# RainBoltz/smore

Hardware: AMD Instinct MI355X
Metric: M edge-updates/sec (d=64, neg=5) (higher is better)
Workload: dtype f32; 1 GPU; LINE order-2 sampled negative-sampling SGD, config c4; vertices=10000000, edge_slots=400000000, dim=64, negative=5, scatter=hybrid, scatter_asked=hybrid, sync=none, parallelism=replicas1

## Files before the change

include/smore_hip.h:

```cpp
#ifndef SMORE_HIP_H
#define SMORE_HIP_H

#include <stddef.h>
#include <stdint.h>

#ifdef __cplusplus
extern "C" {
#endif

typedef struct smore_ctx smore_ctx;

#define SMORE_OK 0
#define SMORE_EINVAL 1
#define SMORE_EHIP 2
#define SMORE_ENOMEM 3
#define SMORE_ESTATE 4
#define SMORE_EIO 5

#define SMORE_VM_OUT_DEGREES 0
#define SMORE_VM_NO_DEGREES 1
#define SMORE_VM_DEGREES 2
#define SMORE_NM_DEGREES 0
#define SMORE_NM_IN_DEGREES 1
#define SMORE_NM_NO_DEGREES 2
// ... 58 lines not shown

int smore_train_edges_async(smore_ctx* ctx, int model, uint64_t begin, uint64_t count,
                            uint64_t total, int K, double alpha0, double reg, uint64_t seed,
                            int mode);
int smore_train_edges(smore_ctx* ctx, int model, uint64_t begin, uint64_t count,
                      uint64_t total, int K, double alpha0, double reg, uint64_t seed,
                      int mode);
int smore_set_hot_threshold(smore_ctx* ctx, double tau);
int smore_set_write_combine(smore_ctx* ctx, int rows, int flush_rounds);
int smore_write_combine_info(const smore_ctx* ctx, int* rows, int* flush_rounds);
int smore_hot_rows(const smore_ctx* ctx, int64_t* hot_w, int64_t* hot_c);
int smore_hot_row_ids(smore_ctx* ctx, int model, int K, int which, int64_t n, int32_t* ids);
int smore_skipped(smore_ctx* ctx, uint64_t* skipped);
float smore_last_kernel_ms(const smore_ctx* ctx);
int smore_last_mode(const smore_ctx* ctx);
int smore_copy_bandwidth(smore_ctx* ctx, uint64_t bytes, int reps, double* gbs);
int smore_last_phase_ms(const smore_ctx* ctx, float* draw_ms, float* update_ms, int* launches);

int smore_delta_begin(smore_ctx* ctx, const void* T, void* S, void* D, void* R, int64_t n);
int smore_delta_end(smore_ctx* ctx, void* T, void* S, const void* D, const void* R, float scale, int64_t n);
int smore_delta_cycle(smore_ctx* ctx, void* T, void* S, void* D, void* R, float scale, int64_t n);
int smore_delta_end_rows(smore_ctx* ctx, void* T, void* S, const void* D, const void* R, const void* scale,
                         int64_t rows, int64_t stride);
int smore_delta_cycle_rows(smore_ctx* ctx, void* T, void* S, void* D, void* R, const void* scale, int64_t rows,
                           int64_t stride);
int smore_source_parts(smore_ctx* ctx, int nparts, int64_t* bounds);
int smore_set_source_partition(smore_ctx* ctx, int nparts, int part);
int smore_row_rates(smore_ctx* ctx, int model, int K, int which, int64_t n, double* rate);
#define SMORE_SYNC_SUM 0
#define SMORE_SYNC_MEAN 1
// ... 194 lines not shown
```

smore_amd/_lib.py:

```python
import ctypes as C
import os

HERE = os.path.dirname(os.path.abspath(__file__))
LIB_PATH = os.environ.get("SMORE_LIB") or os.path.join(HERE, "lib", "libsmore_hip.so")

OK, EINVAL, EHIP, ENOMEM, ESTATE, EIO = range(6)
VM = {"out_degrees": 0, "no_degrees": 1, "degrees": 2}
NM = {"degrees": 0, "in_degrees": 1, "no_degrees": 2}
AT_VERTEX, AT_NEGATIVE, AT_CONTEXT = 0, 1, 2
W, CTX = 0, 1
MODEL = {"line2": 0, "line1": 1, "mf": 2, "bpr": 3, "census": 16}
SYNC = {"sum": 0, "mean": 1, "adaptive": 2}


def sync_rule(sync):
    if isinstance(sync, bool):
        return int(sync)
    return SYNC[sync]


MODE = {"hogwild": 0, "atomic": 1, "serial": 2, "hybrid": 3}
SCHED = {"replicas": 0, "blocks": 1}
SEM = {"cpp": 0, "go": 1}

# ... 35 lines not shown
        "smore_get_table": (i32, [P, i32, P, i64, i32]),
        "smore_table_device": (i32, [P, i32, C.POINTER(P), C.POINTER(i64)]),
        "smore_train_edges_async": (i32, [P, i32, u64, u64, u64, i32, dbl, dbl, u64, i32]),
        "smore_train_edges": (i32, [P, i32, u64, u64, u64, i32, dbl, dbl, u64, i32]),
        "smore_skipped": (i32, [P, C.POINTER(u64)]),
        "smore_set_hot_threshold": (i32, [P, dbl]),
        "smore_set_semantics": (i32, [P, i32]),
        "smore_set_write_combine": (i32, [P, i32, i32]),
        "smore_write_combine_info": (i32, [P, C.POINTER(i32), C.POINTER(i32)]),
        "smore_gen_powerlaw": (i32, [i64, i64, i32, dbl, u64, P, P]),
        "smore_hot_rows": (i32, [P, C.POINTER(i64), C.POINTER(i64)]),
        "smore_hot_row_ids": (i32, [P, i32, i32, i32, i64, P]),
        "smore_group_set_hot_exchange": (i32, [P, i64, i32]),
        "smore_last_kernel_ms": (C.c_float, [P]),
        "smore_last_mode": (i32, [P]),
        "smore_copy_bandwidth": (i32, [P, u64, i32, C.POINTER(C.c_double)]),
        "smore_last_phase_ms": (i32, [P, C.POINTER(C.c_float), C.POINTER(C.c_float), C.POINTER(i32)]),
        "smore_delta_begin": (i32, [P, P, P, P, P, i64]),
        "smore_delta_end": (i32, [P, P, P, P, P, C.c_float, i64]),
        "smore_delta_cycle": (i32, [P, P, P, P, P, C.c_float, i64]),
        "smore_delta_end_rows": (i32, [P, P, P, P, P, P, i64, i64]),
        "smore_delta_cycle_rows": (i32, [P, P, P, P, P, P, i64, i64]),
        "smore_row_rates": (i32, [P, i32, i32, i32, i64, P]),
        "smore_source_parts": (i32, [P, i32, P]),
        "smore_set_source_partition": (i32, [P, i32, i32]),
        "smore_exchange_set_adaptive": (i32, [P, i32, i32, dbl, dbl]),
        "smore_group_set_adaptive": (i32, [P, dbl]),
        "smore_group_set_partition": (i32, [P, i32]),
        "smore_group_set_walk_partition": (i32, [P, i32]),
        "smore_train_deepwalk": (i32, [P, u64, u64, i32, i32, i32, i32, dbl, u64, P, i32]),
# ... 118 lines not shown
```

smore_amd/csrc/capi.cpp:

```cpp
#include "hot_exchange.h"
#include "train_host.h"

#include <algorithm>
#include <chrono>
#include <cmath>
#include <cstdio>
#include <cstdlib>
#include <cstring>
#include <limits>
#include <string>
#include <vector>

using namespace smore_host;

extern "C" {

const char* smore_version(void) { return "smore_hip 0.1 (gfx950)"; }

int smore_create(int device, smore_ctx** out) {
    if (!out) return SMORE_EINVAL;
    *out = nullptr;
    smore_ctx* c = new smore_ctx();
    c->device = device;
    if (device < 0) {
// ... 19 lines not shown
}

void smore_destroy(smore_ctx* c) {
    if (!c) return;
    smore_exchange_release(c);
    if (c->device >= 0) {
        (void)hipSetDevice(c->device);
        (void)hipStreamSynchronize(c->stream);
    }
    dfree(c->d_offsets); dfree(c->d_targets); dfree(c->d_vtab); dfree(c->d_ntab); dfree(c->d_ctab);
    dfree(c->d_sig); dfree(c->d_skipped); dfree(c->d_work); dfree(c->d_warp_stats); dfree(c->d_field); dfree(c->d_hoprec_slots); dfree(c->d_hoprec_stats); dfree(c->d_skewopt_stats);
    dfree(c->d_table[0]); dfree(c->d_table[1]);

    dfree(c->d_order); dfree(c->d_walks); dfree(c->d_lens); dfree(c->d_tcum); dfree(c->d_wts); dfree(c->d_nbr_sorted); dfree(c->d_ntype); dfree(c->d_ttargets); dfree(c->d_toff); dfree(c->d_paths); dfree(c->d_path_off); dfree(c->d_t_off); dfree(c->d_t_tgt); dfree(c->d_t_ts); dfree(c->d_t_min); dfree(c->d_t_max); dfree(c->d_sh_hash); dfree(c->d_sh_ids);
    dfree(c->d_rec); dfree(c->d_vt32); dfree(c->d_ct16); dfree(c->d_split);
    dfree(c->d_pcount); dfree(c->d_poff); dfree(c->d_pairs); dfree(c->d_census[0]); dfree(c->d_census[1]);
    dfree(c->d_io_ids[0]); dfree(c->d_io_rows[0]); dfree(c->d_io_ids[1]); dfree(c->d_io_rows[1]);
    blocks_release(c);
    if (c->d_scan_tmp) (void)hipFree(c->d_scan_tmp);
    for (hipEvent_t e : c->phase_ev) (void)hipEventDestroy(e);
    if (c->ev0) (void)hipEventDestroy(c->ev0);
    if (c->ev1) (void)hipEventDestroy(c->ev1);
    if (c->own_stream) (void)hipStreamDestroy(c->own_stream);
    if (c->draw_stream) (void)hipStreamDestroy(c->draw_stream);
    for (hipEvent_t e : c->sync_ev) (void)hipEventDestroy(e);
    delete c;
}

const char* smore_last_error(const smore_ctx* c) { return c ? c->err.c_str() : "null context"; }

// ... 333 lines not shown
            if (e == hipSuccess) e = hipEventSynchronize(c->ev1);
            float ms = 0.0f;
            if (e == hipSuccess) e = hipEventElapsedTime(&ms, c->ev0, c->ev1);
            if (e == hipSuccess && ms > 0) best = std::max(best, 2.0 * (double)n16 * 16 * reps / (ms * 1e-3) / 1e9);
        }
    (void)hipFree(src);
    (void)hipFree(dst);
    c->timed = false;
    if (e != hipSuccess) return fail(c, SMORE_EHIP, hipGetErrorString(e));
    *gbs = best;
    return SMORE_OK;
}

int smore_last_mode(const smore_ctx* c) { return c ? c->last_mode : -1; }

float smore_last_kernel_ms(const smore_ctx* c) {
    if (!c || !c->timed) return -1.0f;
    float ms = -1.0f;
    if (hipEventSynchronize(c->ev1) != hipSuccess) return -1.0f;
    if (hipEventElapsedTime(&ms, c->ev0, c->ev1) != hipSuccess) return -1.0f;
    return ms;
}

int smore_deepwalk_order(int64_t V, int walk_times, uint64_t skip, int64_t* order) {
    if (V <= 0 || walk_times < 0 || !order) return SMORE_EINVAL;
    deepwalk_order(V, walk_times, skip, order);
    return SMORE_OK;
}

int smore_load_pretrain(smore_ctx* c, int which, const char* path) {
// ... 224 lines not shown
```

smore_amd/csrc/ctx.h:

```cpp
#pragma once
#include <hip/hip_runtime.h>

#include <algorithm>
#include <array>
#include <cmath>
#include <cstdlib>
#include <cstring>
#include <memory>
#include <string>
#include <vector>

#include "../../include/smore_hip.h"
#include "host_graph.h"
#include "train_kernels.h"

using namespace smore;

struct smore_ctx {
    int device = 0;
    hipStream_t stream = nullptr;
    hipStream_t own_stream = nullptr;
    hipStream_t draw_stream = nullptr;
    std::vector<hipEvent_t> sync_ev;
    std::string err;
// ... 56 lines not shown
    int32_t* d_t_tgt = nullptr;
    double* d_t_ts = nullptr;
    double* d_t_min = nullptr;
    double* d_t_max = nullptr;
    double t_min_time = 0.0, t_max_time = 0.0;
    bool has_temporal = false;
    int2* d_sh_hash = nullptr;
    int32_t* d_sh_ids = nullptr;
    int sh_rows = 0;
    int sh_max = 128, sh_flush = 0;
    int sh_flush_eff = 32;
    int sh_flush_w_eff = 0;
    int sh_lvl_eff[8] = {0, 0, 0, 0, 0, 0, 0, 0};
    int32_t* d_rec = nullptr;
    unsigned long long* d_split = nullptr;
    uint32_t* d_pcount = nullptr;
    uint64_t* d_poff = nullptr;
    size_t pair_walks = 0;
    void* d_scan_tmp = nullptr;
    size_t scan_tmp_bytes = 0;
    uint4* d_vt32 = nullptr;
    uint4* d_ct16 = nullptr;
    bool packed_ok = false;
    size_t rec_cap = 0;
    std::vector<hipEvent_t> phase_ev;
    int phase_n = 0;
    void* comm = nullptr;
    bool own_comm = false;
    bool local_comm = false;
    int nranks = 1, rank = 0;
// ... 213 lines not shown
```

smore_amd/csrc/edge_inst.h:

```cpp
#pragma once
#include "edge_kernels.h"

namespace smore {

template <int KMAX, int MODE>
const void* edge_symbol(int dpad, int model) {
    const int G = lanes_of(dpad), M = regs_of(dpad);
#define X(g, m)                                                                          \
    if (G == g && M == m) {                                                              \
        if (model == SMORE_BPR) {                                                        \
            if constexpr (KMAX == 5) return (const void*)edge_train_kernel<g, m, 5, MODE, 2>; \
            else return nullptr;                                                         \
        }                                                                                \
        return model == SMORE_LINE2 ? (const void*)edge_train_kernel<g, m, KMAX, MODE, 0> \
                                    : (const void*)edge_train_kernel<g, m, KMAX, MODE, 1>; \
    }
    SMORE_FOR_EACH_GM(X)
#undef X
    return nullptr;
}

template <int KMAX, int MODE>
const void* pair_symbol(int dpad, int) {
    const int G = lanes_of(dpad), M = regs_of(dpad);
// ... 9 lines not shown
```

smore_amd/csrc/edge_kernels.h:

```cpp
#pragma once
#include "train_kernels.h"

namespace smore {

#ifndef SMORE_WAVES_STORE
#define SMORE_WAVES_STORE 0
#endif
#ifndef SMORE_WAVES_ATOMIC
#define SMORE_WAVES_ATOMIC 0
#endif
#ifndef SMORE_WAVES_HYBRID
#define SMORE_WAVES_HYBRID 3
#endif
#ifndef SMORE_WAVES_BPR
#define SMORE_WAVES_BPR 0
#endif
constexpr int waves_of(int mode, int shared = 0) {
    return shared == 2 ? SMORE_WAVES_BPR
                       : mode == MODE_STORE ? SMORE_WAVES_STORE : mode == MODE_ATOMIC ? SMORE_WAVES_ATOMIC : SMORE_WAVES_HYBRID;
}

template <int MODE>
__device__ __forceinline__ bool scatter_atomic(int32_t tagged) {
    if constexpr (MODE == MODE_ATOMIC) return true;
// ... 461 lines not shown
        if (!(key & SH_WKEY)) continue;
        const float x = atomicExch(&sh.pend[i], 0.0f);
        if (x != 0.0f) unsafeAtomicAdd(Tw + (int64_t)(key & ~SH_WKEY) * dpad + (i - s * dpad), x);
    }
}

__device__ __forceinline__ float neg_scale_of(const EdgeArgs& a, uint64_t count) {
    if (a.neg_lo && a.neg_hi) {
        const uint64_t tot = *a.neg_hi - *a.neg_lo;
        return count > 0 && tot > 0 && a.neg_scale > 0.0f
                   ? (float)((double)a.neg_scale * (double)tot / (double)count) : 1.0f;
    }
    return a.neg_scale > 0.0f ? a.neg_scale : 1.0f;
}

template <int G, int M, int KMAX, int MODE, int SHARED>
__global__ void __launch_bounds__(256) __attribute__((amdgpu_waves_per_eu(waves_of(MODE, SHARED))))
edge_train_kernel(EdgeArgs a) {
    __shared__ float s_sig[1001];
    extern __shared__ float s_dyn[];
    int32_t* sh_ids = nullptr;
    const ShState sh = block_setup<MODE>(a, s_sig, s_dyn, sh_ids);

    const int lane = threadIdx.x & (G - 1);
    uint64_t rb = a.rec_base ? *a.rec_base : 0;
    uint64_t count = (a.count_dev ? *a.count_dev : a.count) - rb;
    const float nsc = neg_scale_of(a, count);
    if (a.part_n > 1) {
        const uint64_t lo = count * a.part_q / a.part_n, hi = count * (a.part_q + 1) / a.part_n;
        rb += lo;
        count = hi - lo;
    }
    const int32_t* const recs = a.rec + rb * (uint64_t)rec_width(KMAX);
// ... 103 lines not shown
#pragma unroll
            for (int q = 0; q < RW / 4; ++q) r[q] = i32x4{-1, -1, -1, -1};
            if (t < lim) {
                const i32x4* p = reinterpret_cast<const i32x4*>(recs + t * RW);
#pragma unroll
                for (int q = 0; q < RW / 4; ++q) r[q] = __builtin_nontemporal_load(p + q);
            }
        };
        i32x4 rr[RW / 4];
        Ids xa, xb;
        float wva[M], rowsa[KMAX + 1][M], wvb[M], rowsb[KMAX + 1][M];
        __shared__ uint64_t s_next;
        uint64_t ch_rounds = count / ((uint64_t)gridDim.x * gpb * 16u);
        ch_rounds = ch_rounds < 8 ? 8 : ch_rounds > CH_ROUNDS ? CH_ROUNDS : ch_rounds;
        if (a.pair_slice && !a.alpha_rec) ch_rounds = a.pair_slice;
        const uint64_t span = ch_rounds * gpb;
        auto grab = [&]() -> uint64_t {
            __syncthreads();
            if (threadIdx.x == 0) s_next = atomicAdd(a.work, 1ull) * span;
            __syncthreads();
            return s_next;
        };
        for (uint64_t c0 = grab(); c0 < count; c0 = grab()) {
            const uint64_t lim = c0 + span < count ? c0 + span : count;
            if constexpr (SHARED == 2) {
                uint64_t t = c0 + gib;
                load_rec(t, lim, rr);
                for (uint64_t r = c0; r < lim; r += gpb) {
                    t = r + gib;
                    decode(t, lim, rr, xa);
// ... 1 lines not shown
                    if (xa.live) {
                        int32_t id[KMAX + 1];
                        bool hot[KMAX + 1];
                        xa.ids(id);
                        xa.hots(hot);
                        gather_rows<G, M, KMAX>(a, lane, ev, xa.v(), id, shared, wva, rowsa);
                        if constexpr (KMAX == 5)
                            bpr_update_rows<G, M, KMAX, MODE>(a, s_sig, lane, ev, xa.v(), id,
                                                              scatter_atomic<MODE>(xa.w[0]), hot, xa.alpha, wva, rowsa,
                                                              sh);
                    }
                    maybe_flush();
                }
                continue;
            }
            uint64_t t = c0 + gib;
            load_rec(t, lim, rr);
            decode(t, lim, rr, xa);
            {
                int32_t id[KMAX + 1];
                xa.ids(id);
                gather_rows<G, M, KMAX>(a, lane, ev, xa.v(), id, shared, wva, rowsa);
            }
            load_rec(t + gpb, lim, rr);
            for (uint64_t r = c0; r < lim; r += gpb) {
                t = r + gib;
                decode(t + gpb, lim, rr, xb);
                load_rec(t + 2 * gpb, lim, rr);
                {
                    int32_t id[KMAX + 1];
// ... 153 lines not shown
```

smore_amd/csrc/train.cpp:

```cpp
#include "train_host.h"

#include <algorithm>
#include <cstdlib>
#include <cstring>
#include <string>
#include <thread>
#include <vector>

using namespace smore_host;

namespace smore_host {

int edge_grid(smore_ctx* c, const UpdateKernel& k, int mode, uint64_t count, bool leave_slot) {
    if (mode == SMORE_SERIAL) return 1;
    int per_cu = 0;
    if (!k.fn || hipOccupancyMaxActiveBlocksPerMultiprocessor(&per_cu, k.fn, 256, k.lds) != hipSuccess || per_cu < 1)
        per_cu = 1;
    if (leave_slot && per_cu > 1) per_cu -= 1;
    if (const char* e = getenv("SMORE_BLOCKS_PER_CU")) {
        const int cap = atoi(e);
        if (cap > 0 && cap < per_cu) per_cu = cap;
    }
    int64_t grid = (int64_t)c->cus * per_cu;
    if (const char* e = getenv("SMORE_MAX_BLOCKS")) {
// ... 140 lines not shown
        } else {
            a.K = K;
        }
    }
    if (model == SMORE_BPR && !go && mode == SMORE_HYBRID) {
        const char* e = getenv("SMORE_BPR_SCATTER");
        EdgeArgs t = a;
        t.sh_rows = 0;
        const int64_t Mb = (int64_t)edge_grid(c, UpdateFamily::Cpp, t) * (256 / lanes_of(c->dpad));
        const bool small = c->hot_tau < 0 && 16.0 * (double)Mb >= (double)c->g->V;
        if (!small && !(e && !strcmp(e, "tagged"))) a.mode = mode = SMORE_HOGWILD;
    }
    const char* bpr_comb = getenv("SMORE_BPR_COMBINE");
    const bool combine = mode == SMORE_HYBRID && (go || model != SMORE_BPR || (bpr_comb && atoi(bpr_comb) != 0));
    const int hot_model = go && model == SMORE_BPR ? SMORE_LINE2 : model;
    int grid;
    if ((rc = plan_record_launch(c, a, combine, fam, hot_model, go ? HOT_TAU_WALK : HOT_TAU_EDGE,
                                 EDGE_FLUSH_MAX, &grid)))
        return rc;
    const int RW = rec_width(kmax_of(a.K));
    uint64_t chunk_max = (uint64_t)1 << 27;
    if (const char* e = getenv("SMORE_DRAW_CHUNK")) chunk_max = std::max<uint64_t>(1024, strtoull(e, nullptr, 10));
    if (a.mode == SMORE_SERIAL) chunk_max = ((uint64_t)1 << 30) / (uint64_t)RW;
    const uint64_t chunk = std::min<uint64_t>(count, chunk_max);
    const int nch = (int)((count + chunk - 1) / chunk);
    const int nbuf = nch > 1 ? 2 : 1;
    if ((rc = ensure_cap(c, c->d_rec, c->rec_cap, chunk * RW * nbuf))) return rc;
    if ((rc = grow_events(c, c->phase_ev, 2 * (size_t)nch + 1))) return rc;
    if ((rc = grow_events(c, c->sync_ev, 2 * (size_t)nch))) return rc;
    if ((rc = ensure_packed(c))) return rc;
    const DevGraph dg = dev_graph(c);
    const bool split = mode == SMORE_HYBRID && !go && dg.vt32 && split_on();
    if (split && !c->d_split) HIPCHK(c, hipMalloc((void**)&c->d_split, 4 * sizeof(unsigned long long)));
    const char* leave_env = getenv("SMORE_DRAW_LEAVE");
    const bool leave = !leave_env || atoi(leave_env) != 0;
    const int ugrid = nch > 1 ? edge_grid(c, fam, a, leave) : grid;
    hipStream_t ds = nch > 1 ? c->draw_stream : c->stream;
    auto recbuf = [&](int k) { return c->d_rec + (size_t)(k % nbuf) * chunk * RW; };
    auto draw = [&](int k) -> int {
        const uint64_t b = (uint64_t)k * chunk, n = std::min<uint64_t>(chunk, count - b);
        if (k >= 2) HIPCHK(c, hipStreamWaitEvent(ds, c->sync_ev[2 * (k - 2) + 1], 0));
        if (go) HIPCHK(c, launch_go_draw(dg, c->d_tcum, c->go_unit_w, seed, begin + b, n, a.K, recbuf(k), c->d_skipped, ds));
        else if (split) {
            unsigned long long* cnt = c->d_split + 2 * (k % nbuf);
            HIPCHK(c, hipMemsetAsync(cnt, 0, 2 * sizeof(unsigned long long), ds));
            HIPCHK(c, launch_draw_split(dg, seed, begin + b, n, a.K, alpha0, total,
                                        model == SMORE_MF || model == SMORE_BPR ? 0 : 1, recbuf(k), c->d_skipped, cnt,
                                        ds));
        } else HIPCHK(c, launch_draw(dg, seed, begin + b, n, a.K, recbuf(k), c->d_skipped, ds));
        HIPCHK(c, hipEventRecord(c->sync_ev[2 * k], ds));
        return SMORE_OK;
    };
    HIPCHK(c, hipEventRecord(c->ev0, c->stream));
    HIPCHK(c, hipEventRecord(c->phase_ev[0], c->stream));
    if (ds != c->stream) HIPCHK(c, hipStreamWaitEvent(ds, c->phase_ev[0], 0));
    if ((rc = draw(0))) return rc;
    for (int k = 0; k < nch; ++k) {
        if (k + 1 < nch && (rc = draw(k + 1))) return rc;
        HIPCHK(c, hipStreamWaitEvent(c->stream, c->sync_ev[2 * k], 0));
        HIPCHK(c, hipEventRecord(c->phase_ev[2 * k + 1], c->stream));
        const uint64_t b = (uint64_t)k * chunk, n = std::min<uint64_t>(chunk, count - b);
        EdgeArgs ak = a;
        ak.begin = begin + b;
        ak.count = n;
        ak.rec = recbuf(k);
        HIPCHK(c, hipMemsetAsync(c->d_work, 0, sizeof(unsigned long long), c->stream));
        if (split) {
            unsigned long long* cnt = c->d_split + 2 * (k % nbuf);
            ak.alpha_rec = 2;
            ak.count_dev = reinterpret_cast<const uint64_t*>(cnt);
            HIPCHK(c, launch_update(update_kernel(fam, ak), ak, ugrid, c->stream));
            EdgeArgs ac = ak;
            ac.mode = SMORE_HOGWILD;
            ac.sh_rows = 0;
            ac.count_dev = nullptr;
            ac.rec_base = reinterpret_cast<const uint64_t*>(cnt);
            HIPCHK(c, hipMemsetAsync(c->d_work, 0, sizeof(unsigned long long), c->stream));
            HIPCHK(c, launch_update(update_kernel(fam, ac), ac, edge_grid(c, fam, ac), c->stream));
        } else HIPCHK(c, launch_update(update_kernel(fam, ak), ak, ugrid, c->stream));
        HIPCHK(c, hipEventRecord(c->phase_ev[2 * k + 2], c->stream));
// ... 429 lines not shown
```

smore_amd/csrc/train_kernels.h:

```cpp
#pragma once
#include <hip/hip_runtime.h>

#include <algorithm>
#include <cstdlib>

#include "../../include/smore_hip.h"
#include "device_common.h"

namespace smore {

enum { MODE_STORE = SMORE_HOGWILD, MODE_ATOMIC = SMORE_ATOMIC, MODE_HYBRID = SMORE_HYBRID };

struct EdgeArgs {
    DevGraph g;
    const float* sig;
    float* W;
    float* C;
    unsigned long long* skipped;
    const double* tcum;
    const int2* sh_hash;
    const int32_t* sh_ids;
    int sh_rows, sh_flush;
    int sh_flush_w;
    int sh_lvl[8];
    const int32_t* rec;
    const uint64_t* count_dev;
    const uint64_t* rec_base;
    unsigned long long* work;
    int alpha_rec;
    uint32_t pair_slice;
    float neg_scale;
    const uint64_t* neg_lo;
    const uint64_t* neg_hi;
    int w_plain;
    uint32_t part_q, part_n;
    int rec_edge;
    int w_comb;
    uint64_t begin, count, total, seed;
    double alpha0;
    float reg;
    int dpad, K, model, mode;
};

struct WalkArgs {
    const int64_t* order;
    uint64_t order_base;
    int32_t* walks;
    int32_t* lens;
    uint64_t walk_begin, nwalks, total_walks;
    int steps, window;
    int rule;
    int window_min;
// ... 16 lines not shown
    int sample_times;
    double jump;
};

int lanes_of(int dpad);
inline int regs_of(int dpad) {
    const int G = lanes_of(dpad);
    return 4 * ((dpad / 4 + G - 1) / G);
}
constexpr int rec_width(int kmax) {
    int r = 4;
    while (r < 2 + kmax) r <<= 1;
    return r;
}
constexpr uint64_t CH_ROUNDS = 128;
inline int kmax_of(int K) { return K <= 5 ? 5 : K <= 10 ? 10 : 20; }
hipError_t launch_delta_begin(const float* T, float* S, float* D, float* R, uint64_t n, int cus, hipStream_t st);
hipError_t launch_delta_end(float* T, float* S, const float* D, const float* R, float scale, uint64_t n, int cus,
                            hipStream_t st);
hipError_t launch_delta_cycle(float* T, float* S, float* D, float* R, float scale, uint64_t n, int cus,
                              hipStream_t st);
hipError_t launch_pair_count(const WalkArgs& w, uint64_t seed, uint32_t* count, hipStream_t st);
inline uint64_t pair_bound(int steps, int window, int rule = 0, int window_min = 0) {
    const uint64_t L = (uint64_t)steps + 1;
    if (rule == 1) return L * 2 * (uint64_t)std::max(1, window - window_min + 1);
    const uint64_t r = std::min<uint64_t>(2 * (uint64_t)window, L - 1);
    return L * r;
}
hipError_t scan_pair_counts(const uint32_t* count, uint64_t* off, uint64_t n, void** temp, size_t* temp_bytes,
                            hipStream_t st);
hipError_t launch_pair_emit(const DevGraph& g, const WalkArgs& w, uint64_t seed, int K, double alpha0,
                            const uint64_t* off, int32_t* rec, hipStream_t st);
hipError_t launch_pack(const DevGraph& g, uint64_t E, uint4* vt32, uint4* ct16, hipStream_t st);
hipError_t launch_draw_split(const DevGraph& g, uint64_t seed, uint64_t begin, uint64_t count, int K, double alpha0,
                             uint64_t total, int base, int32_t* rec, unsigned long long* skipped,
                             unsigned long long* counts, hipStream_t st);
hipError_t launch_draw(const DevGraph& g, uint64_t seed, uint64_t begin, uint64_t count, int K, int32_t* rec,
                       unsigned long long* skipped, hipStream_t st);
constexpr int SH_HASH = 256;
constexpr int32_t SH_WKEY = 1 << 30;
inline int sh_rows_max(int dpad) {
    static const int lds = [] {
        const char* e = getenv("SMORE_SH_LDS");
        const int v = e ? atoi(e) : 8192;
        return v > 0 ? v : 8192;
    }();
    const int r = lds / (dpad > 0 ? dpad : 1);
    return r < SH_HASH - 1 ? r : SH_HASH - 1;
}

inline size_t sh_lds_bytes(int sh_rows, int dpad) {
    return sh_rows > 0 ? SH_HASH * 8 + (size_t)sh_rows * 4 + (size_t)sh_rows * dpad * 4 : 0;
}
// ... 83 lines not shown
    X(Edge, MODE_ATOMIC, 5) X(Edge, MODE_ATOMIC, 10) X(Edge, MODE_ATOMIC, 20)       \
    X(Edge, MODE_HYBRID, 5) X(Edge, MODE_HYBRID, 10) X(Edge, MODE_HYBRID, 20)       \
    X(Pair, MODE_STORE, 5) X(Pair, MODE_STORE, 10)                                  \
    X(Pair, MODE_ATOMIC, 5) X(Pair, MODE_ATOMIC, 10)                                \
    X(Pair, MODE_HYBRID, 5) X(Pair, MODE_HYBRID, 10)                                \
    X(GoRec, MODE_STORE, 5) X(GoRec, MODE_STORE, 10)                                \
    X(GoRec, MODE_ATOMIC, 5) X(GoRec, MODE_ATOMIC, 10)                              \
    X(GoRec, MODE_HYBRID, 5) X(GoRec, MODE_HYBRID, 10)                              \
    X(GoPair, MODE_STORE, 5) X(GoPair, MODE_STORE, 10)                              \
    X(GoPair, MODE_ATOMIC, 5) X(GoPair, MODE_ATOMIC, 10)                            \
    X(GoPair, MODE_HYBRID, 5) X(GoPair, MODE_HYBRID, 10)                            \
    X(Warp, WARP_STORE, WARP_KMAX) X(Warp, WARP_ATOMIC, WARP_KMAX)                  \
    X(HopRec, MODE_STORE, HOPREC_KMAX) X(HopRec, MODE_ATOMIC, HOPREC_KMAX)          \
    X(SkewOpt, MODE_STORE, SKEWOPT_KMAX) X(SkewOpt, MODE_ATOMIC, SKEWOPT_KMAX)

template <KernelFamily F, int MODE, int KMAX>
const void* update_symbol(int dpad, int model);
#define X(F, MODE, KMAX) \
    template <>          \
    const void* update_symbol<KernelFamily::F, MODE, KMAX>(int dpad, int model);
SMORE_FOR_EACH_UPDATE_KERNEL(X)
#undef X
#define SMORE_UPDATE_INST(F, MODE, KMAX, ladder)                                          \
    namespace smore {                                                                     \
    template <>                                                                           \
    const void* update_symbol<KernelFamily::F, MODE, KMAX>(int dpad, int model) {         \
        return ladder<KMAX, MODE>(dpad, model);                                           \
    }                                                                                     \
    }

// ... 53 lines not shown
```

smore_amd/csrc/train_kernels.hip:

```cpp

#include "train_kernels.h"

namespace smore {

__global__ void sample_kernel(DevGraph g, uint64_t seed, uint64_t begin, uint64_t count, int K,
                              int bpr, int32_t* out) {
    const uint64_t t = (uint64_t)blockIdx.x * blockDim.x + threadIdx.x;
    if (t >= count) return;
    const uint64_t s = begin + t;
    const int nslot = bpr ? 14 : 4 + 2 * K;
    const int width = bpr ? 7 : 2 + K;
    int32_t* o = out + t * width;
    uint32_t w[4];
    uint32_t blk = 0xFFFFFFFFu;
    auto word = [&](int j) -> uint32_t {
        if ((uint32_t)(j >> 2) != blk) {
            blk = (uint32_t)(j >> 2);
            const uint4 b = philox_block(seed, 0, s, blk);
            w[0] = b.x; w[1] = b.y; w[2] = b.z; w[3] = b.w;
        }
        return w[j & 3];
    };
    (void)nslot;
    const int32_t v = untag(source_sample(g, word(0), word(1)));
// ... 38 lines not shown
    return nullptr;
}

static bool pair_path(const EdgeArgs& a) {
    return a.alpha_rec == 1 && a.mode != SMORE_SERIAL && a.K <= 10 && !a.rec_edge;
}

UpdateKernel update_kernel(UpdateFamily f, const EdgeArgs& a) {
    KernelFamily kf = KernelFamily::Edge;
    int kmax = kmax_of(a.K);
    switch (f) {
        case UpdateFamily::Cpp: kf = pair_path(a) ? KernelFamily::Pair : KernelFamily::Edge; break;
        case UpdateFamily::GoRec: kf = KernelFamily::GoRec; kmax = std::min(kmax, 10); break;
        case UpdateFamily::GoPair: kf = KernelFamily::GoPair; kmax = std::min(kmax, 10); break;
    }
    return {find_symbol(kf, a.mode, kmax, a.dpad, a.model),
            a.mode == SMORE_HYBRID ? sh_lds_bytes(a.sh_rows, a.dpad) : 0};
}

UpdateKernel update_kernel(const WarpArgs& a) {
    const int mode = a.mode == SMORE_ATOMIC ? SMORE_ATOMIC : SMORE_HOGWILD;
    return {find_symbol(KernelFamily::Warp, mode, WARP_KMAX, a.dpad, 0), 0};
}

UpdateKernel update_kernel(const HopRecArgs& a) {
    const int mode = a.mode == SMORE_ATOMIC ? SMORE_ATOMIC : SMORE_HOGWILD;
    return {find_symbol(KernelFamily::HopRec, mode, HOPREC_KMAX, a.dpad, 0), 0};
}

UpdateKernel update_kernel(const SkewOptArgs& a) {
    const int mode = a.mode == SMORE_ATOMIC ? SMORE_ATOMIC : SMORE_HOGWILD;
// ... 22 lines not shown
```

smore_amd/pronet.py:

```python
import ctypes as C

import numpy as np

from . import _lib
from ._lib import check, lib, ptr


class ProNet:

    def __init__(self, device=0, _ctx=None):
        self.ctx = C.c_void_p()
        self._owned = _ctx is None
        if _ctx is not None:
            self.ctx = C.c_void_p(_ctx)
        else:
            rc = lib.smore_create(int(device), C.byref(self.ctx))
            if rc != _lib.OK:
                raise _lib.SmoreError("smore_create(device=%d) failed with status %d" % (device, rc))
        self.device = device
        self.vertex_method = "out_degrees"
        self.negative_method = "degrees"
        self.dim = 0

    def close(self):
# ... 493 lines not shown
    def synchronize(self):
        self._chk(lib.smore_synchronize(self.ctx), "synchronize")

    def skipped(self):
        s = C.c_uint64()
        self._chk(lib.smore_skipped(self.ctx, C.byref(s)), "skipped")
        return s.value

    def last_kernel_ms(self):
        return float(lib.smore_last_kernel_ms(self.ctx))

    def last_mode(self):
        m = int(lib.smore_last_mode(self.ctx))
        return {v: k for k, v in _lib.MODE.items()}.get(m)

    def delta_begin(self, T, S, D, R, n):
        self._chk(lib.smore_delta_begin(self.ctx, T, S, D, R, int(n)), "delta_begin")

    def delta_end(self, T, S, D, R, scale, n):
        self._chk(lib.smore_delta_end(self.ctx, T, S, D, R, float(scale), int(n)), "delta_end")

    def delta_cycle(self, T, S, D, R, scale, n):
        self._chk(lib.smore_delta_cycle(self.ctx, T, S, D, R, float(scale), int(n)), "delta_cycle")

    def delta_end_rows(self, T, S, D, R, scale, rows, stride):
        self._chk(lib.smore_delta_end_rows(self.ctx, T, S, D, R, scale, int(rows), int(stride)), "delta_end_rows")

    def delta_cycle_rows(self, T, S, D, R, scale, rows, stride):
        self._chk(lib.smore_delta_cycle_rows(self.ctx, T, S, D, R, scale, int(rows), int(stride)),
                  "delta_cycle_rows")
# ... 201 lines not shown
```

Measured before the change: 1340 M edge-updates/s.

## Draw edge samples grouped by source vertex and reuse source rows across runs

Adds an ordered draw path that bucket-sorts the sampled edges by source vertex before writing edge records. It is built from a count, scan, scatter and a per-tile local sort. A new RUNS variant of the LINE2 edge kernel then keeps the source embedding row in registers while consecutive records share a source. It writes that row back once per run, either as a store or as an atomic delta, and forwards just-updated context rows to the next record when they match. This aims to cut repeated gathers and scatters of W rows in hybrid mode, at the price of extra sort kernels and scratch buffers in the draw stage and a changed update order.

Result: slower. 1251 M edge-updates/s (-6.6%).

```diff
diff --git a/include/smore_hip.h b/include/smore_hip.h
--- a/include/smore_hip.h
+++ b/include/smore_hip.h
@@ -96,6 +96,9 @@
 int smore_skipped(smore_ctx* ctx, uint64_t* skipped);
 float smore_last_kernel_ms(const smore_ctx* ctx);
 int smore_last_mode(const smore_ctx* ctx);
+int smore_set_source_order(smore_ctx* ctx, int mode);
+int smore_last_source_order(const smore_ctx* ctx);
+int smore_edge_records_copy(smore_ctx* ctx, int32_t* out, uint64_t words);
 int smore_copy_bandwidth(smore_ctx* ctx, uint64_t bytes, int reps, double* gbs);
 int smore_last_phase_ms(const smore_ctx* ctx, float* draw_ms, float* update_ms, int* launches);
 
diff --git a/smore_amd/_lib.py b/smore_amd/_lib.py
--- a/smore_amd/_lib.py
+++ b/smore_amd/_lib.py
@@ -73,6 +73,9 @@
         "smore_group_set_hot_exchange": (i32, [P, i64, i32]),
         "smore_last_kernel_ms": (C.c_float, [P]),
         "smore_last_mode": (i32, [P]),
+        "smore_set_source_order": (i32, [P, i32]),
+        "smore_last_source_order": (i32, [P]),
+        "smore_edge_records_copy": (i32, [P, P, u64]),
         "smore_copy_bandwidth": (i32, [P, u64, i32, C.POINTER(C.c_double)]),
         "smore_last_phase_ms": (i32, [P, C.POINTER(C.c_float), C.POINTER(C.c_float), C.POINTER(i32)]),
         "smore_delta_begin": (i32, [P, P, P, P, P, i64]),
diff --git a/smore_amd/csrc/capi.cpp b/smore_amd/csrc/capi.cpp
--- a/smore_amd/csrc/capi.cpp
+++ b/smore_amd/csrc/capi.cpp
@@ -57,6 +57,7 @@
 
     dfree(c->d_order); dfree(c->d_walks); dfree(c->d_lens); dfree(c->d_tcum); dfree(c->d_wts); dfree(c->d_nbr_sorted); dfree(c->d_ntype); dfree(c->d_ttargets); dfree(c->d_toff); dfree(c->d_paths); dfree(c->d_path_off); dfree(c->d_t_off); dfree(c->d_t_tgt); dfree(c->d_t_ts); dfree(c->d_t_min); dfree(c->d_t_max); dfree(c->d_sh_hash); dfree(c->d_sh_ids);
     dfree(c->d_rec); dfree(c->d_vt32); dfree(c->d_ct16); dfree(c->d_split);
+    dfree(c->d_ord_key); dfree(c->d_ord_list); dfree(c->d_ord_cnt);
     dfree(c->d_pcount); dfree(c->d_poff); dfree(c->d_pairs); dfree(c->d_census[0]); dfree(c->d_census[1]);
     dfree(c->d_io_ids[0]); dfree(c->d_io_rows[0]); dfree(c->d_io_ids[1]); dfree(c->d_io_rows[1]);
     blocks_release(c);
@@ -420,6 +421,25 @@
 
 int smore_last_mode(const smore_ctx* c) { return c ? c->last_mode : -1; }
 
+int smore_set_source_order(smore_ctx* c, int mode) {
+    if (!c) return SMORE_EINVAL;
+    if (mode < -1 || mode > 1) return fail(c, SMORE_EINVAL, "source order: -1 automatic, 0 off, 1 on");
+    c->src_order = mode;
+    return SMORE_OK;
+}
+
+int smore_last_source_order(const smore_ctx* c) { return c ? (c->src_ran ? 1 : 0) : -1; }
+
+int smore_edge_records_copy(smore_ctx* c, int32_t* out, uint64_t words) {
+    if (!c || !out) return SMORE_EINVAL;
+    if (!c->d_rec || words > c->rec_cap) return fail(c, SMORE_EINVAL, "edge records: more words than the buffer holds");
+    int rc;
+    if ((rc = set_device(c))) return rc;
+    HIPCHK(c, hipStreamSynchronize(c->stream));
+    HIPCHK(c, hipMemcpy(out, c->d_rec, words * sizeof(int32_t), hipMemcpyDeviceToHost));
+    return SMORE_OK;
+}
+
 float smore_last_kernel_ms(const smore_ctx* c) {
     if (!c || !c->timed) return -1.0f;
     float ms = -1.0f;
diff --git a/smore_amd/csrc/ctx.h b/smore_amd/csrc/ctx.h
--- a/smore_amd/csrc/ctx.h
+++ b/smore_amd/csrc/ctx.h
@@ -94,6 +94,12 @@
     int sh_lvl_eff[8] = {0, 0, 0, 0, 0, 0, 0, 0};
     int32_t* d_rec = nullptr;
     unsigned long long* d_split = nullptr;
+    int src_order = -1;
+    bool src_ran = false;
+    uint32_t* d_ord_key = nullptr;
+    uint32_t* d_ord_list = nullptr;
+    uint32_t* d_ord_cnt = nullptr;
+    size_t ord_key_cap = 0, ord_list_cap = 0, ord_cnt_cap = 0;
     uint32_t* d_pcount = nullptr;
     uint64_t* d_poff = nullptr;
     size_t pair_walks = 0;
diff --git a/smore_amd/csrc/edge_inst.h b/smore_amd/csrc/edge_inst.h
--- a/smore_amd/csrc/edge_inst.h
+++ b/smore_amd/csrc/edge_inst.h
@@ -6,8 +6,12 @@
 template <int KMAX, int MODE>
 const void* edge_symbol(int dpad, int model) {
     const int G = lanes_of(dpad), M = regs_of(dpad);
+    const bool runs = (model & MODEL_SRC_RUNS) != 0;
+    model &= ~MODEL_SRC_RUNS;
+    if (runs && model != SMORE_LINE2) return nullptr;
 #define X(g, m)                                                                          \
     if (G == g && M == m) {                                                              \
+        if (runs) return (const void*)edge_train_kernel<g, m, KMAX, MODE, 0, true>;      \
         if (model == SMORE_BPR) {                                                        \
             if constexpr (KMAX == 5) return (const void*)edge_train_kernel<g, m, 5, MODE, 2>; \
             else return nullptr;                                                         \
diff --git a/smore_amd/csrc/edge_kernels.h b/smore_amd/csrc/edge_kernels.h
--- a/smore_amd/csrc/edge_kernels.h
+++ b/smore_amd/csrc/edge_kernels.h
@@ -499,9 +499,10 @@
     return a.neg_scale > 0.0f ? a.neg_scale : 1.0f;
 }
 
-template <int G, int M, int KMAX, int MODE, int SHARED>
+template <int G, int M, int KMAX, int MODE, int SHARED, bool RUNS = false>
 __global__ void __launch_bounds__(256) __attribute__((amdgpu_waves_per_eu(waves_of(MODE, SHARED))))
 edge_train_kernel(EdgeArgs a) {
+    static_assert(!RUNS || SHARED == 0, "W_v stays in registers only with two tables");
     __shared__ float s_sig[1001];
     extern __shared__ float s_dyn[];
     int32_t* sh_ids = nullptr;
@@ -635,6 +636,7 @@
         uint64_t ch_rounds = count / ((uint64_t)gridDim.x * gpb * 16u);
         ch_rounds = ch_rounds < 8 ? 8 : ch_rounds > CH_ROUNDS ? CH_ROUNDS : ch_rounds;
         if (a.pair_slice && !a.alpha_rec) ch_rounds = a.pair_slice;
+        if constexpr (RUNS) ch_rounds = a.src_rounds;
         const uint64_t span = ch_rounds * gpb;
         auto grab = [&]() -> uint64_t {
             __syncthreads();
@@ -666,6 +668,96 @@
                 }
                 continue;
             }
+            if constexpr (RUNS) {
+                float wv0[M];
+                uint64_t t = c0 + gib;
+                load_rec(t, lim, rr);
+                decode(t, lim, rr, xa);
+                {
+                    int32_t id[KMAX + 1];
+                    xa.ids(id);
+                    gather_rows<G, M, KMAX>(a, lane, ev, xa.v(), id, false, wva, rowsa);
+                }
+#pragma unroll
+                for (int m = 0; m < M; ++m) wv0[m] = wva[m];
+                bool edge = true;
+                int run = 1;
+                float fwd[M];
+                int fwd_kind = 0;
+#pragma unroll
+                for (int m = 0; m < M; ++m) fwd[m] = 0.0f;
+                load_rec(t + gpb, lim, rr);
+                for (uint64_t r = c0; r < lim; r += gpb) {
+                    t = r + gib;
+                    decode(t + gpb, lim, rr, xb);
+                    load_rec(t + 2 * gpb, lim, rr);
+                    const bool same = xa.live && xb.live && xa.w[0] == xb.w[0] && !tag_hot(xa.w[0]);
+                    const bool cont = same && run < SRC_RUN_MAX;
+                    {
+                        int32_t id[KMAX + 1];
+                        xb.ids(id);
+                        gather_ctx_rows<G, M, KMAX>(a, lane, ev, id, rowsb);
+                        const int32_t vb = xb.v();
+                        ld_row<G, M>(wvb, a.W + (int64_t)(vb < 0 ? 0 : vb) * a.dpad, lane, ev, vb >= 0 && !same);
+                    }
+                    if (xa.live) {
+                        int32_t id[KMAX + 1];
+                        bool hot[KMAX + 1];
+                        xa.ids(id);
+                        xa.hots(hot);
+                        if (fwd_kind != 0) {
+                            const bool comb = MODE == MODE_HYBRID && fwd_kind == 2 && sh.n > 0 && hot[0] &&
+                                              sh_lookup(sh.hash, id[0]) >= 0;
+#pragma unroll
+                            for (int m = 0; m < M; ++m)
+                                rowsa[0][m] = fwd_kind == 1 ? fwd[m] : comb ? rowsa[0][m] : rowsa[0][m] + fwd[m];
+                        }
+                        sgd_update_rows<G, M, KMAX, MODE, 0, false>(a, s_sig, lane, ev, xa.v(), id, false, hot, xa.alpha,
+                                                                    false, false, sh, wva, rowsa, false, nsc);
+                        fwd_kind = 0;
+                        if (xb.live) {
+                            const int32_t cb = untag(xb.w[1]);
+#pragma unroll
+                            for (int k = 0; k <= KMAX; ++k)
+                                if (id[k] == cb) {
+                                    constexpr bool DELTA = MODE == MODE_ATOMIC || MODE == MODE_HYBRID;
+                                    const bool dk = DELTA && hot[k];
+                                    const bool add = dk && fwd_kind == 2;
+#pragma unroll
+                                    for (int m = 0; m < M; ++m) fwd[m] = add ? fwd[m] + rowsa[k][m] : rowsa[k][m];
+                                    fwd_kind = dk ? 2 : 1;
+                                }
+                        }
+                        if (!cont) {
+                            float* const wq = a.W + (int64_t)xa.v() * a.dpad;
+                            if (MODE == MODE_ATOMIC || edge || t + gpb >= lim || scatter_atomic<MODE>(xa.w[0])) {
+                                float d[M];
+#pragma unroll
+                                for (int m = 0; m < M; ++m) d[m] = wva[m] - wv0[m];
+                                atomic_row<G, M>(wq, d, lane, a.dpad);
+                            } else {
+                                st_row<G, M>(wq, wva, lane, ev);
+                            }
+                        }
+                    }
+                    if (!same) {
+#pragma unroll
+                        for (int m = 0; m < M; ++m) wva[m] = wv0[m] = wvb[m];
+                        edge = false;
+                    } else if (!cont) {
+#pragma unroll
+                        for (int m = 0; m < M; ++m) wv0[m] = wva[m];
+                    }
+                    run = cont ? run + 1 : 1;
+                    xa = xb;
+#pragma unroll
+                    for (int m = 0; m < M; ++m)
+#pragma unroll
+                        for (int k = 0; k <= KMAX; ++k) rowsa[k][m] = rowsb[k][m];
+                    maybe_flush();
+                }
+                continue;
+            }
             uint64_t t = c0 + gib;
             load_rec(t, lim, rr);
             decode(t, lim, rr, xa);
diff --git a/smore_amd/csrc/train.cpp b/smore_amd/csrc/train.cpp
--- a/smore_amd/csrc/train.cpp
+++ b/smore_amd/csrc/train.cpp
@@ -178,15 +178,25 @@
     const char* bpr_comb = getenv("SMORE_BPR_COMBINE");
     const bool combine = mode == SMORE_HYBRID && (go || model != SMORE_BPR || (bpr_comb && atoi(bpr_comb) != 0));
     const int hot_model = go && model == SMORE_BPR ? SMORE_LINE2 : model;
-    int grid;
-    if ((rc = plan_record_launch(c, a, combine, fam, hot_model, go ? HOT_TAU_WALK : HOT_TAU_EDGE,
-                                 EDGE_FLUSH_MAX, &grid)))
-        return rc;
     const int RW = rec_width(kmax_of(a.K));
     uint64_t chunk_max = (uint64_t)1 << 27;
     if (const char* e = getenv("SMORE_DRAW_CHUNK")) chunk_max = std::max<uint64_t>(1024, strtoull(e, nullptr, 10));
     if (a.mode == SMORE_SERIAL) chunk_max = ((uint64_t)1 << 30) / (uint64_t)RW;
     const uint64_t chunk = std::min<uint64_t>(count, chunk_max);
+    const bool ordered = !go && model == SMORE_LINE2 && a.mode != SMORE_SERIAL &&
+                         c->g->E < ((int64_t)1 << 32) && !split_on() &&
+                         chunk < ((uint64_t)1 << 32) && c->src_order != 0 &&
+                         (c->src_order == 1 ||
+                          (a.mode == SMORE_HYBRID && chunk >= 2 * (uint64_t)c->g->V &&
+                           chunk <= 32 * (uint64_t)c->g->V && chunk >= ((uint64_t)1 << 24)));
+    const char* runs_env = getenv("SMORE_SRC_RUNS");
+    const bool runs = ordered && !(runs_env && atoi(runs_env) == 0);
+    a.src_rounds = runs ? 1 : 0;
+    a.alpha_rec = ordered ? 2 : 0;
+    int grid;
+    if ((rc = plan_record_launch(c, a, combine, fam, hot_model, go ? HOT_TAU_WALK : HOT_TAU_EDGE,
+                                 EDGE_FLUSH_MAX, &grid)))
+        return rc;
     const int nch = (int)((count + chunk - 1) / chunk);
     const int nbuf = nch > 1 ? 2 : 1;
     if ((rc = ensure_cap(c, c->d_rec, c->rec_cap, chunk * RW * nbuf))) return rc;
@@ -201,6 +211,18 @@
     const int ugrid = nch > 1 ? edge_grid(c, fam, a, leave) : grid;
     hipStream_t ds = nch > 1 ? c->draw_stream : c->stream;
     auto recbuf = [&](int k) { return c->d_rec + (size_t)(k % nbuf) * chunk * RW; };
+    const uint32_t gpb = 256 / (uint32_t)lanes_of(c->dpad);
+    auto rounds_of = [&](uint64_t n) {
+        const uint64_t r = n / ((uint64_t)ugrid * gpb * 16u);
+        return (uint32_t)(r < 8 ? 8 : r > CH_ROUNDS ? CH_ROUNDS : r);
+    };
+    if (ordered) {
+        if (!dg.vt32) return fail(c, SMORE_ESTATE, "source order: no packed draw tables");
+        if ((rc = ensure_cap(c, c->d_ord_key, c->ord_key_cap, (size_t)chunk))) return rc;
+        if ((rc = ensure_cap(c, c->d_ord_list, c->ord_list_cap, (size_t)chunk))) return rc;
+        if ((rc = ensure_cap(c, c->d_ord_cnt, c->ord_cnt_cap, ((size_t)3 << order_bits(chunk, dg.V)) + 1))) return rc;
+    }
+    c->src_ran = ordered;
     auto draw = [&](int k) -> int {
         const uint64_t b = (uint64_t)k * chunk, n = std::min<uint64_t>(chunk, count - b);
         if (k >= 2) HIPCHK(c, hipStreamWaitEvent(ds, c->sync_ev[2 * (k - 2) + 1], 0));
@@ -211,6 +233,10 @@
             HIPCHK(c, launch_draw_split(dg, seed, begin + b, n, a.K, alpha0, total,
                                         model == SMORE_MF || model == SMORE_BPR ? 0 : 1, recbuf(k), c->d_skipped, cnt,
                                         ds));
+        } else if (ordered) {
+            HIPCHK(c, launch_draw_ordered(dg, seed, begin + b, n, a.K, alpha0, total, 1, gpb, rounds_of(n) * gpb,
+                                          order_bits(n, dg.V), c->d_ord_key, c->d_ord_list, c->d_ord_cnt, recbuf(k),
+                                          c->d_skipped, c->cus, ds));
         } else HIPCHK(c, launch_draw(dg, seed, begin + b, n, a.K, recbuf(k), c->d_skipped, ds));
         HIPCHK(c, hipEventRecord(c->sync_ev[2 * k], ds));
         return SMORE_OK;
@@ -228,6 +254,7 @@
         ak.begin = begin + b;
         ak.count = n;
         ak.rec = recbuf(k);
+        ak.src_rounds = runs ? rounds_of(n) : 0;
         HIPCHK(c, hipMemsetAsync(c->d_work, 0, sizeof(unsigned long long), c->stream));
         if (split) {
             unsigned long long* cnt = c->d_split + 2 * (k % nbuf);
diff --git a/smore_amd/csrc/train_draw_order.hip b/smore_amd/csrc/train_draw_order.hip
--- /dev/null
+++ b/smore_amd/csrc/train_draw_order.hip
@@ -0,0 +1,226 @@
+#include "train_kernels.h"
+
+namespace smore {
+
+__device__ __forceinline__ uint32_t order_bucket(uint32_t y, int bits) { return bits ? y >> (32 - bits) : 0u; }
+
+int order_bits(uint64_t n, uint32_t V) {
+    int bits = 0;
+    auto fits = [&](int b) {
+        const double mean = (double)(n >> b);
+        return mean + 8.0 * __builtin_sqrt(mean) + 1.0 <= (double)ORD_TILE && (uint64_t)(V >> b) + 3 <= ORD_KEYS / 2;
+    };
+    while (bits < ORD_BITS_MAX && !fits(bits)) ++bits;
+    return bits;
+}
+
+__global__ void __launch_bounds__(ORD_BLOCK) order_count_kernel(uint64_t seed, uint64_t begin, uint32_t n, int bits,
+                                                                uint32_t* key, uint32_t* cnt) {
+    __shared__ uint32_t s_h[ORD_HIST];
+    const uint32_t B = 1u << bits;
+    const bool lds = B <= (uint32_t)ORD_HIST;
+    if (lds) {
+        for (uint32_t i = threadIdx.x; i < B; i += ORD_BLOCK) s_h[i] = 0u;
+        __syncthreads();
+    }
+    const uint64_t lo = (uint64_t)n * blockIdx.x / gridDim.x, hi = (uint64_t)n * (blockIdx.x + 1) / gridDim.x;
+    for (uint64_t i = lo + threadIdx.x; i < hi; i += ORD_BLOCK) {
+        const uint32_t y = philox_block(seed, 0, begin + i, 0).y;
+        key[i] = y;
+        const uint32_t b = order_bucket(y, bits);
+        if (lds) atomicAdd(&s_h[b], 1u);
+        else atomicAdd(&cnt[b], 1u);
+    }
+    if (lds) {
+        __syncthreads();
+        for (uint32_t i = threadIdx.x; i < B; i += ORD_BLOCK) {
+            const uint32_t x = s_h[i];
+            if (x) atomicAdd(&cnt[i], x);
+        }
+    }
+}
+
+__device__ __forceinline__ uint32_t order_block_scan(uint32_t* s, uint32_t x) {
+    s[threadIdx.x] = x;
+    __syncthreads();
+    for (uint32_t d = 1; d < (uint32_t)ORD_BLOCK; d <<= 1) {
+        const uint32_t v = threadIdx.x >= d ? s[threadIdx.x - d] : 0u;
+        __syncthreads();
+        s[threadIdx.x] += v;
+        __syncthreads();
+    }
+    return s[threadIdx.x];
+}
+
+__global__ void __launch_bounds__(ORD_BLOCK) order_scan_kernel(const uint32_t* cnt, uint32_t* start, uint32_t* cursor,
+                                                               uint32_t B) {
+    __shared__ uint32_t s_sum[ORD_BLOCK];
+    const uint32_t per = (B + ORD_BLOCK - 1) / ORD_BLOCK;
+    const uint32_t lo = threadIdx.x * per < B ? threadIdx.x * per : B, hi = lo + per < B ? lo + per : B;
+    uint32_t s = 0;
+    for (uint32_t i = lo; i < hi; ++i) s += cnt[i];
+    uint32_t run = order_block_scan(s_sum, s) - s;
+    for (uint32_t i = lo; i < hi; ++i) {
+        start[i] = run;
+        cursor[i] = run;
+        run += cnt[i];
+    }
+    if (threadIdx.x == ORD_BLOCK - 1) start[B] = s_sum[ORD_BLOCK - 1];
+}
+
+__global__ void __launch_bounds__(ORD_BLOCK) order_scatter_kernel(const uint32_t* key, uint32_t n, int bits,
+                                                                  uint32_t* cursor, uint32_t* list) {
+    __shared__ uint32_t s_h[ORD_HIST];
+    const uint32_t B = 1u << bits;
+    const uint64_t lo = (uint64_t)n * blockIdx.x / gridDim.x, hi = (uint64_t)n * (blockIdx.x + 1) / gridDim.x;
+    if (B > (uint32_t)ORD_HIST) {
+        for (uint64_t i = lo + threadIdx.x; i < hi; i += ORD_BLOCK)
+            list[atomicAdd(&cursor[order_bucket(key[i], bits)], 1u)] = (uint32_t)i;
+        return;
+    }
+    for (uint32_t i = threadIdx.x; i < B; i += ORD_BLOCK) s_h[i] = 0u;
+    __syncthreads();
+    for (uint64_t i = lo + threadIdx.x; i < hi; i += ORD_BLOCK) atomicAdd(&s_h[order_bucket(key[i], bits)], 1u);
+    __syncthreads();
+    for (uint32_t i = threadIdx.x; i < B; i += ORD_BLOCK) {
+        const uint32_t x = s_h[i];
+        s_h[i] = x ? atomicAdd(&cursor[i], x) : 0u;
+    }
+    __syncthreads();
+    for (uint64_t i = lo + threadIdx.x; i < hi; i += ORD_BLOCK)
+        list[atomicAdd(&s_h[order_bucket(key[i], bits)], 1u)] = (uint32_t)i;
+}
+
+__device__ __forceinline__ uint32_t ordered_slot(uint32_t P, uint32_t n, uint32_t gpb, uint32_t span) {
+    const uint32_t c0 = P / span * span, p = P - c0;
+    const uint32_t m = n - c0 < span ? n - c0 : span;
+    const uint32_t rf = m / gpb, rem = m - rf * gpb, head = rem * (rf + 1);
+    uint32_t g, r;
+    if (p < head) {
+        g = p / (rf + 1);
+        r = p - g * (rf + 1);
+    } else {
+        const uint32_t q = p - head;
+        g = q / rf;
+        r = q - g * rf;
+        g += rem;
+    }
+    return c0 + r * gpb + g;
+}
+
+template <int KMAX>
+__global__ void __launch_bounds__(ORD_BLOCK) __attribute__((amdgpu_waves_per_eu(KMAX == 5 ? 8 : 4))) ordered_draw_kernel(DevGraph g, uint64_t seed, uint64_t begin, uint32_t n,
+                                                                 int K, int bits, const uint32_t* start,
+                                                                 const uint32_t* list, double alpha0, uint64_t total,
+                                                                 int base, uint32_t gpb, uint32_t span, int32_t* rec,
+                                                                 unsigned long long* skipped) {
+    constexpr int RW = rec_width(KMAX);
+    static_assert(RW > 2 + KMAX, "a record needs a free word for the rate");
+    __shared__ uint32_t s_cnt[ORD_KEYS];
+    __shared__ uint32_t s_key[ORD_TILE];
+    __shared__ uint32_t s_sum[ORD_BLOCK];
+    const uint32_t lo = start[blockIdx.x], hi = start[blockIdx.x + 1];
+    const uint32_t slot_lo = draw_index(bits ? blockIdx.x << (32 - bits) : 0u, g.V);
+    for (uint32_t t0 = lo; t0 < hi; t0 += ORD_TILE) {
+        const uint32_t m = hi - t0 < (uint32_t)ORD_TILE ? hi - t0 : (uint32_t)ORD_TILE;
+        for (uint32_t i = threadIdx.x; i < (uint32_t)ORD_KEYS; i += ORD_BLOCK) s_cnt[i] = 0u;
+        __syncthreads();
+        for (uint32_t i = threadIdx.x; i < m; i += ORD_BLOCK) {
+            const uint4 b0 = philox_block(seed, 0, begin + list[t0 + i], 0);
+            const uint32_t vi = draw_index(b0.y, g.V);
+            const uint32_t thr = g.vt32[2 * (uint64_t)vi].x;
+            uint32_t k = 2u * (vi - slot_lo) + (b0.x < thr ? 0u : 1u);
+            k = k < (uint32_t)ORD_KEYS ? k : (uint32_t)ORD_KEYS - 1u;
+            s_key[i] = k | (atomicAdd(&s_cnt[k], 1u) << 16);
+        }
+        __syncthreads();
+        {
+            constexpr int PER = ORD_KEYS / ORD_BLOCK;
+            uint32_t x[PER], s = 0;
+#pragma unroll
+            for (int j = 0; j < PER; ++j) s += x[j] = s_cnt[threadIdx.x * PER + j];
+            uint32_t run = order_block_scan(s_sum, s) - s;
+#pragma unroll
+            for (int j = 0; j < PER; ++j) {
+                s_cnt[threadIdx.x * PER + j] = run;
+                run += x[j];
+            }
+        }
+        __syncthreads();
+        for (uint32_t i = threadIdx.x; i < m; i += ORD_BLOCK) {
+            const uint32_t off = list[t0 + i], kr = s_key[i];
+            const uint32_t P = t0 + s_cnt[kr & 0xFFFFu] + (kr >> 16);
+            const uint64_t s = begin + off;
+            const uint4 b0 = philox_block(seed, 0, s, 0);
+            const uint32_t vi = draw_index(b0.y, g.V);
+            const uint4 p0 = g.vt32[2 * (uint64_t)vi], p1 = g.vt32[2 * (uint64_t)vi + 1];
+            uint32_t nidx[KMAX], np[KMAX];
+#pragma unroll
+            for (int j = 0; j < KMAX; j += 2) {
+                if (j < K) {
+                    const uint4 b = philox_block(seed, 0, s, 1 + j / 2);
+                    nidx[j] = draw_index(b.x, g.V);
+                    np[j] = b.y;
+                    if (j + 1 < KMAX) {
+                        nidx[j + 1] = draw_index(b.z, g.V);
+                        np[j + 1] = b.w;
+                    }
+                }
+            }
+            uint2 ne[KMAX];
+#pragma unroll
+            for (int j = 0; j < KMAX; ++j)
+                if (j < K) ne[j] = g.ntab[nidx[j]];
+            const bool acc = b0.x < p0.x;
+            const int32_t tv = alias_pick(vi, make_uint2(p0.x, p0.y), b0.x);
+            const uint32_t eo = acc ? p0.z : p1.x, br = acc ? p0.w : p1.y;
+            int32_t c = -1;
+            if (br != 0) {
+                const uint4 ce = g.ct16[(uint64_t)eo + draw_index(b0.w, br)];
+                c = b0.z < ce.x ? (int32_t)ce.z : (int32_t)ce.y;
+            }
+            int32_t w[RW];
+            w[0] = tv;
+            w[1] = c;
+#pragma unroll
+            for (int j = 0; j < RW - 2; ++j) w[2 + j] = (j < KMAX && j < K) ? alias_pick(nidx[j], ne[j], np[j]) : -1;
+            w[2 + KMAX] = __float_as_int(alpha_at(s + (uint64_t)base, alpha0, total));
+            i32x4* o = reinterpret_cast<i32x4*>(rec + (uint64_t)ordered_slot(P, n, gpb, span) * RW);
+#pragma unroll
+            for (int q = 0; q < RW / 4; ++q) {
+                const i32x4 x = {w[4 * q], w[4 * q + 1], w[4 * q + 2], w[4 * q + 3]};
+                __builtin_nontemporal_store(x, o + q);
+            }
+            if (c < 0) atomicAdd(skipped, 1ull);
+        }
+        __syncthreads();
+    }
+}
+
+hipError_t launch_draw_ordered(const DevGraph& g, uint64_t seed, uint64_t begin, uint64_t count, int K, double alpha0,
+                               uint64_t total, int base, uint32_t gpb, uint32_t span, int bits, uint32_t* key,
+                               uint32_t* list, uint32_t* cnt, int32_t* rec, unsigned long long* skipped, int cus,
+                               hipStream_t st) {
+    const uint32_t n = (uint32_t)count, B = 1u << bits;
+    uint32_t* const start = cnt + B;
+    uint32_t* const cursor = start + B + 1;
+    hipError_t e = hipMemsetAsync(cnt, 0, (size_t)B * sizeof(uint32_t), st);
+    if (e != hipSuccess) return e;
+    const uint64_t need = (count + ORD_BLOCK - 1) / ORD_BLOCK;
+    const dim3 grid((unsigned)std::max<uint64_t>(1, std::min<uint64_t>(need, 2 * (uint64_t)std::max(1, cus))));
+    hipLaunchKernelGGL(order_count_kernel, grid, dim3(ORD_BLOCK), 0, st, seed, begin, n, bits, key, cnt);
+    hipLaunchKernelGGL(order_scan_kernel, dim3(1), dim3(ORD_BLOCK), 0, st, cnt, start, cursor, B);
+    hipLaunchKernelGGL(order_scatter_kernel, grid, dim3(ORD_BLOCK), 0, st, key, n, bits, cursor, list);
+#define SMORE_DRAW(KM)                                                                                              \
+    hipLaunchKernelGGL((ordered_draw_kernel<KM>), dim3(B), dim3(ORD_BLOCK), 0, st, g, seed, begin, n, K, bits, start, \
+                       list, alpha0, total, base, gpb, span, rec, skipped);
+    switch (kmax_of(K)) {
+        case 5: SMORE_DRAW(5) break;
+        case 10: SMORE_DRAW(10) break;
+        default: SMORE_DRAW(20) break;
+    }
+#undef SMORE_DRAW
+    return hipGetLastError();
+}
+
+}
diff --git a/smore_amd/csrc/train_kernels.h b/smore_amd/csrc/train_kernels.h
--- a/smore_amd/csrc/train_kernels.h
+++ b/smore_amd/csrc/train_kernels.h
@@ -36,6 +36,7 @@
     uint32_t part_q, part_n;
     int rec_edge;
     int w_comb;
+    uint32_t src_rounds;
     uint64_t begin, count, total, seed;
     double alpha0;
     float reg;
@@ -82,6 +83,7 @@
     return r;
 }
 constexpr uint64_t CH_ROUNDS = 128;
+constexpr int SRC_RUN_MAX = 32;
 inline int kmax_of(int K) { return K <= 5 ? 5 : K <= 10 ? 10 : 20; }
 hipError_t launch_delta_begin(const float* T, float* S, float* D, float* R, uint64_t n, int cus, hipStream_t st);
 hipError_t launch_delta_end(float* T, float* S, const float* D, const float* R, float scale, uint64_t n, int cus,
@@ -105,6 +107,16 @@
                              unsigned long long* counts, hipStream_t st);
 hipError_t launch_draw(const DevGraph& g, uint64_t seed, uint64_t begin, uint64_t count, int K, int32_t* rec,
                        unsigned long long* skipped, hipStream_t st);
+constexpr int ORD_BLOCK = 1024;
+constexpr int ORD_TILE = 10240;
+constexpr int ORD_KEYS = 4096;
+constexpr int ORD_HIST = 16384;
+constexpr int ORD_BITS_MAX = 24;
+int order_bits(uint64_t n, uint32_t V);
+hipError_t launch_draw_ordered(const DevGraph& g, uint64_t seed, uint64_t begin, uint64_t count, int K, double alpha0,
+                               uint64_t total, int base, uint32_t gpb, uint32_t span, int bits, uint32_t* key,
+                               uint32_t* list, uint32_t* cnt, int32_t* rec, unsigned long long* skipped, int cus,
+                               hipStream_t st);
 constexpr int SH_HASH = 256;
 constexpr int32_t SH_WKEY = 1 << 30;
 inline int sh_rows_max(int dpad) {
@@ -218,6 +230,7 @@
     X(HopRec, MODE_STORE, HOPREC_KMAX) X(HopRec, MODE_ATOMIC, HOPREC_KMAX)          \
     X(SkewOpt, MODE_STORE, SKEWOPT_KMAX) X(SkewOpt, MODE_ATOMIC, SKEWOPT_KMAX)
 
+constexpr int MODEL_SRC_RUNS = 0x100;
 template <KernelFamily F, int MODE, int KMAX>
 const void* update_symbol(int dpad, int model);
 #define X(F, MODE, KMAX) \
diff --git a/smore_amd/csrc/train_kernels.hip b/smore_amd/csrc/train_kernels.hip
--- a/smore_amd/csrc/train_kernels.hip
+++ b/smore_amd/csrc/train_kernels.hip
@@ -76,7 +76,9 @@
         case UpdateFamily::GoRec: kf = KernelFamily::GoRec; kmax = std::min(kmax, 10); break;
         case UpdateFamily::GoPair: kf = KernelFamily::GoPair; kmax = std::min(kmax, 10); break;
     }
-    return {find_symbol(kf, a.mode, kmax, a.dpad, a.model),
+    const bool runs = kf == KernelFamily::Edge && f == UpdateFamily::Cpp && a.model == SMORE_LINE2 && a.src_rounds &&
+                      a.mode != SMORE_SERIAL;
+    return {find_symbol(kf, a.mode, kmax, a.dpad, runs ? a.model | MODEL_SRC_RUNS : a.model),
             a.mode == SMORE_HYBRID ? sh_lds_bytes(a.sh_rows, a.dpad) : 0};
 }
 
diff --git a/smore_amd/pronet.py b/smore_amd/pronet.py
--- a/smore_amd/pronet.py
+++ b/smore_amd/pronet.py
@@ -531,6 +531,21 @@
         m = int(lib.smore_last_mode(self.ctx))
         return {v: k for k, v in _lib.MODE.items()}.get(m)
 
+    def set_source_order(self, mode=-1):
+        self._chk(lib.smore_set_source_order(self.ctx, int(mode)), "set_source_order")
+
+    def last_source_order(self):
+        return int(lib.smore_last_source_order(self.ctx)) == 1
+
+    def edge_records(self, n, K):
+        kmax = 5 if K <= 5 else 10 if K <= 10 else 20
+        rw = 4
+        while rw < 2 + kmax:
+            rw *= 2
+        out = np.zeros((int(n), rw), np.int32)
+        self._chk(lib.smore_edge_records_copy(self.ctx, out.ctypes.data_as(C.c_void_p), out.size), "edge_records")
+        return out
+
     def delta_begin(self, T, S, D, R, n):
         self._chk(lib.smore_delta_begin(self.ctx, T, S, D, R, int(n)), "delta_begin")
 
```
